# traveller59/second.pytorch

Hardware: AMD Instinct MI355X
Metric: frames/sec VoxelNet fwd (car.fhd, ~16k active voxels) (higher is better)
Workload: dtype bf16; 1 GPU; car.fhd.config VoxelNet forward (voxelise+VFE+SpMiddleFHD+RPNV2+rotated NMS), inference, batch=8 synthetic KITTI clouds/GPU (17000 pts, 16000 voxels each), random-init weights, inputs resident in HBM; parallelism=frame-dp1, launch_mode=graph, graph_branches=1, steps_in_flight=4, rpn_segments_serialized=True, rulebook_numbering=sorted, points_per_frame=17000

## Files before the change

second.pytorch_amd/csrc/indice_conv.hip:

```cpp
#include "common.hpp"
#include <stdlib.h>
#include <type_traits>

namespace sec {

template <typename T> struct Cvt;
template <> struct Cvt<float> {
    static __device__ __forceinline__ float to(float v) { return v; }
    static __device__ __forceinline__ float from(float v) { return v; }
};
template <> struct Cvt<__half> {
    static __device__ __forceinline__ float to(__half v) { return __half2float(v); }
    static __device__ __forceinline__ __half from(float v) { return __float2half_rn(v); }
};
template <> struct Cvt<__hip_bfloat16> {
    static __device__ __forceinline__ float to(__hip_bfloat16 v) { return __bfloat162float(v); }
    static __device__ __forceinline__ __hip_bfloat16 from(float v) { return __float2bfloat16(v); }
};

__device__ __forceinline__ float epilogue(float v, const float *scale, const float *shift, int c, int relu) {
    if (scale) v = __fmul_rn(v, scale[c]);
    if (shift) v = __fadd_rn(v, shift[c]);
    if (relu) v = v > 0.0f ? v : 0.0f;
    return v;
// ... 346 lines not shown
            }
            if (valid) store4<OT>(out + (size_t)row * COUT + c0, v[0], v[1], v[2], v[3]);
        }
    }
}

template <typename T, typename OT, int COUT>
__global__ __launch_bounds__(kBlock) void k_conv_c4(const T *__restrict__ feat, const T *__restrict__ w,
                                                   const int *__restrict__ nbr, int n_out,
                                                   const int *__restrict__ num_out_dev, int kvol,
                                                   const float *__restrict__ scale, const float *__restrict__ shift,
                                                   int relu, OT *__restrict__ out) {
    extern __shared__ __attribute__((aligned(16))) float wl[];
    if (num_out_dev) n_out = *num_out_dev;
    for (int e = threadIdx.x; e < kvol * 4 * COUT; e += kBlock) wl[e] = Cvt<T>::to(w[e]);
    __syncthreads();
    long long o = (long long)blockIdx.x * kBlock + threadIdx.x;
    if (o >= n_out) return;
    float acc[COUT];
#pragma unroll
    for (int c = 0; c < COUT; ++c) acc[c] = 0.0f;
    const int *row = nbr + (size_t)o * kvol;
    for (int k = 0; k < kvol; ++k) {
        int idx = row[k];
        if (idx < 0) continue;
        float f[4];
        if (sizeof(T) == 2) {
            uint2 v = *reinterpret_cast<const uint2 *>(feat + (size_t)idx * 4);
            const T *pv = reinterpret_cast<const T *>(&v);
#pragma unroll
            for (int c = 0; c < 4; ++c) f[c] = Cvt<T>::to(pv[c]);
        } else {
            float4 v = *reinterpret_cast<const float4 *>(feat + (size_t)idx * 4);
            f[0] = v.x; f[1] = v.y; f[2] = v.z; f[3] = v.w;
        }
        const float *wk = wl + k * 4 * COUT;
#pragma unroll
        for (int ci = 0; ci < 4; ++ci)
#pragma unroll
            for (int c = 0; c < COUT; ++c) acc[c] = fmaf(f[ci], wk[ci * COUT + c], acc[c]);
    }
    OT *dst = out + (size_t)o * COUT;
#pragma unroll
    for (int c = 0; c < COUT; ++c) dst[c] = Cvt<OT>::from(epilogue(acc[c], scale, shift, c, relu));
}

#ifdef SEC_CONV_EXPERIMENTS
#include "../../tools/kernel_experiments/indice_conv_experiments.inc"
#endif



typedef __attribute__((address_space(3))) void *lds_ptr_c;
typedef const __attribute__((address_space(1))) void *glb_ptr_c;
template <int N> __device__ __forceinline__ void cwait_vmcnt() { asm volatile("s_waitcnt vmcnt(%0)" ::"n"(N) : "memory"); }
__device__ __forceinline__ void clds_barrier() { asm volatile("s_waitcnt lgkmcnt(0)\n\ts_barrier" ::: "memory"); }

template <typename T, int CIN, int COUT>
struct RowsCfg {
    static constexpr int KS = CIN / 16, NT = (COUT + 31) / 32;
    static constexpr int LPR = CIN / 8;
    static constexpr int RPI = 64 / LPR;
    static constexpr int ND = 32 / RPI;
    static constexpr int BPIECES = KS * NT;
    static constexpr int NBW = BPIECES >= 4 ? BPIECES / 4 : 1;
    static constexpr int L = ND + NBW + 1;
    static constexpr int ASLOT = 32 * LPR, BSLOT = BPIECES * 64;
    static constexpr int RING = 3;
};

typedef float f32x2p __attribute__((ext_vector_type(2)));
template <typename T> __device__ __forceinline__ unsigned pack2_16(float a, float b);
template <> __device__ __forceinline__ unsigned pack2_16<__hip_bfloat16>(float a, float b) {
    typedef __bf16 bf16x2p __attribute__((ext_vector_type(2)));
    const f32x2p v = {a, b};
    return __builtin_bit_cast(unsigned, __builtin_convertvector(v, bf16x2p));
}
template <> __device__ __forceinline__ unsigned pack2_16<__half>(float a, float b) {
    typedef _Float16 f16x2p __attribute__((ext_vector_type(2)));
    const f32x2p v = {a, b};
    return __builtin_bit_cast(unsigned, __builtin_convertvector(v, f16x2p));
}

template <typename T, int COUT, bool FUSED>
__device__ __forceinline__ void rows_store_impl(f32x16 (&acc)[(COUT + 31) / 32], T *__restrict__ out, long long row, bool valid, int h,
                                                const float *__restrict__ aff, bool has_scale, bool has_shift, int relu) {
    if (FUSED) { has_scale = has_shift = true; relu = 1; }
    constexpr int NT = (COUT + 31) / 32, NG = COUT >= 32 ? 4 : COUT / 8;
    static_assert(COUT % 16 == 0, "whole 16-byte runs per half-wave pair");
    T *orow = out + (size_t)row * COUT;
    float4 sc4[NT][NG], sh4[NT][NG];
#pragma unroll
    for (int t = 0; t < NT; ++t)
#pragma unroll
        for (int g = 0; g < NG; ++g) {
            const int c = t * 32 + 8 * g + 4 * h;
            if (has_scale) sc4[t][g] = *reinterpret_cast<const float4 *>(aff + c);
            if (has_shift) sh4[t][g] = *reinterpret_cast<const float4 *>(aff + COUT + c);
        }
#pragma unroll
    for (int t = 0; t < NT; ++t) {
        unsigned lo[NG], hi[NG];
#pragma unroll
        for (int g = 0; g < NG; ++g) {
            const float sc[4] = {sc4[t][g].x, sc4[t][g].y, sc4[t][g].z, sc4[t][g].w};
            const float sh[4] = {sh4[t][g].x, sh4[t][g].y, sh4[t][g].z, sh4[t][g].w};
            float v4[4];
#pragma unroll
            for (int j = 0; j < 4; ++j) v4[j] = epilogue_v(acc[t][4 * g + j], sc[j], sh[j], has_scale, has_shift, relu);
            lo[g] = pack2_16<T>(v4[0], v4[1]);
            hi[g] = pack2_16<T>(v4[2], v4[3]);
        }
#pragma unroll
        for (int pr = 0; pr < NG / 2; ++pr) {
            const auto sx = __builtin_amdgcn_permlane32_swap(lo[2 * pr], lo[2 * pr + 1], false, false);
            const auto sy = __builtin_amdgcn_permlane32_swap(hi[2 * pr], hi[2 * pr + 1], false, false);
            if (valid) *reinterpret_cast<uint4 *>(orow + t * 32 + 8 * (2 * pr + h)) = make_uint4(sx[0], sy[0], sx[1], sy[1]);
        }
    }
}
template <typename T, int COUT>
__device__ __forceinline__ void rows_store(f32x16 (&acc)[(COUT + 31) / 32], T *__restrict__ out, long long row, bool valid, int h,
                                           const float *__restrict__ aff, bool has_scale, bool has_shift, int relu) {
    if (has_scale && has_shift && relu) rows_store_impl<T, COUT, true>(acc, out, row, valid, h, aff, true, true, 1);
    else rows_store_impl<T, COUT, false>(acc, out, row, valid, h, aff, has_scale, has_shift, relu);
}

template <int COUT>
__device__ __forceinline__ void rows_stage_affine(float *aff, const float *__restrict__ scale, const float *__restrict__ shift) {
    const int c = threadIdx.x;
    if (c < COUT) {
        if (scale) aff[c] = scale[c];
        if (shift) aff[COUT + c] = shift[c];
    }
}

#ifdef SEC_CONV_TIMELINE
#define SEC_RTL(...) __VA_ARGS__
#else
#define SEC_RTL(...)
#endif

#ifdef SEC_CONV_EXPERIMENTS
#include "../../tools/kernel_experiments/indice_conv_rows_ab.inc"
#endif

typedef unsigned int u32x4_t __attribute__((ext_vector_type(4)));
constexpr int kBalWgs = 256;
#if defined(__HIP_DEVICE_COMPILE__) && defined(SEC_PACKED_F32_EXEMPTION)
#define SEC_PACKED_F32_OK __attribute__((target("packed-fp32-ops")))
#else
#define SEC_PACKED_F32_OK
#endif
template <typename T, int CIN, int COUT, int KVOL, int DIST, int WAVES, int MINW, int FL>
SEC_PACKED_F32_OK __global__ __launch_bounds__(WAVES * 64, MINW) void k_conv_rows_buf(const T *__restrict__ feat, long long feat_bytes,
                                                                   const T *__restrict__ packed, const int *__restrict__ nbr,
                                                                   int n_out, const int *__restrict__ num_out_dev,
                                                                   const float *__restrict__ scale, const float *__restrict__ shift,
                                                                   int relu, T *__restrict__ out) {
    using C = RowsCfg<T, CIN, COUT>;
    constexpr int NBW = (C::BPIECES + WAVES - 1) / WAVES;
    constexpr int ROWB = CIN * (int)sizeof(T);
    constexpr bool STAGE = (FL & 1) != 0, PIPE = (FL & 2) != 0;
    constexpr bool ALLW = (FL & 64) != 0;
    constexpr bool LAZY = (FL & 128) != 0 && STAGE && !ALLW;
    constexpr bool SKEW = (FL & 32) != 0 && WAVES == 8 && PIPE;
    const bool early = SKEW && __builtin_amdgcn_readfirstlane((int)threadIdx.x >> 8) != 0;
    constexpr int TBL16 = 32 * KVOL / 4;
    static_assert(NBW >= 1 && NBW <= 2, "one or two weight pieces per wave");
    static_assert(C::KS <= 4, "up to four 16-channel k-steps per row");
    static_assert(!STAGE || (32 * KVOL) % 4 == 0, "tile table in whole 16-byte pieces");
    static_assert(!ALLW || (STAGE && PIPE), "the all-weights form stages its tables and double-buffers its B fragments");
    constexpr bool WIN3 = (FL & 512) != 0;
    static_assert(!WIN3 || (STAGE && !PIPE && !ALLW && KVOL % 3 == 0 && DIST <= 3), "window form: non-pipelined, 3 offsets per window");
    constexpr int LBUF = ALLW ? (KVOL * C::BSLOT > WAVES * TBL16 ? KVOL * C::BSLOT : WAVES * TBL16) : 1;
    __shared__ __attribute__((aligned(16))) uint4 lbuf[LBUF];
    __shared__ __attribute__((aligned(16))) uint4 bring[ALLW ? 1 : (WIN3 ? 6 : 3)][ALLW ? 1 : C::BSLOT];
    __shared__ __attribute__((aligned(16))) float aff[2 * COUT];
    __shared__ __attribute__((aligned(16))) u32x4_t stage[(STAGE && !ALLW) ? WAVES : 1][(STAGE && !ALLW) ? TBL16 : 1];
    rows_stage_affine<COUT>(aff, scale, shift);
    const int n_cap = n_out;
    if (num_out_dev) n_out = *num_out_dev;
    const int lane = threadIdx.x & 63, w = threadIdx.x >> 6;
    const int r = lane & 31, h = lane >> 5;
    constexpr bool BAL = (FL & 2048) != 0;
    int rw = 32;
    if constexpr (BAL) {
        const int per_wg = (n_out + kBalWgs - 1) / kBalWgs;
        rw = ((per_wg + WAVES - 1) / WAVES + 3) & ~3;
        rw = rw < 4 ? 4 : (rw > 32 ? 32 : rw);
    }
    int bid = blockIdx.x;
    if (relu & 0x10000) {
        const int nact = (int)(((long long)n_out + rw * WAVES - 1) / (rw * WAVES));
        const int per = (nact + 7) >> 3;
        bid = (bid & 7) * per + (bid >> 3);
        if ((int)(blockIdx.x >> 3) >= per) return;
    }
    relu &= 1;
    if ((long long)bid * (rw * WAVES) >= n_out) return;
    const long long row = (long long)bid * (rw * WAVES) + w * rw + r;
    const bool valid = row < n_out && r < rw;
    SEC_RTL(long long *tl = g_timeline; long long tl0 = 0, tl1 = 0, tl2 = 0; if (tl) tl0 = clock64();)
    const __amdgpu_buffer_rsrc_t rsrc = __builtin_amdgcn_make_buffer_rsrc(const_cast<T *>(feat), 0, (int)feat_bytes, 0x00020000);
    const int piece0 = (w * NBW) % C::BPIECES;
    const u32x4_t *wpv = reinterpret_cast<const u32x4_t *>(packed) + (size_t)piece0 * 64 + lane;
    unsigned off[KVOL];
    if constexpr (STAGE) {
        const long long tile_row0 = (long long)bid * (rw * WAVES) + w * rw;
        const long long tbl_bytes = (long long)n_cap * KVOL * 4;
        const int *tile = nbr + tile_row0 * KVOL;
        const long long left = tbl_bytes - tile_row0 * KVOL * 4;
        const __amdgpu_buffer_rsrc_t trs = __builtin_amdgcn_make_buffer_rsrc(
            const_cast<int *>(left > 0 ? tile : nbr), 0, (int)(left <= 0 ? 0 : (left < 32 * KVOL * 4 ? left : 32 * KVOL * 4)), 0x00020000);
        u32x4_t *stg = ALLW ? reinterpret_cast<u32x4_t *>(lbuf) + w * TBL16 : &stage[w][0];
#pragma unroll
        for (int i = 0; i < (TBL16 + 63) / 64; ++i) {
            const int p16 = i * 64 + lane;
            if (p16 < TBL16) stg[p16] = __builtin_amdgcn_raw_buffer_load_b128(trs, p16 * 16, 0, 0);
        }
        __builtin_amdgcn_wave_barrier();
        const int *mine = reinterpret_cast<const int *>(stg) + r * KVOL;
        if constexpr (!LAZY) {
#pragma unroll
            for (int k = 0; k < KVOL; ++k) {
                const int t = valid ? mine[k] : -1;
                off[k] = t >= 0 ? (unsigned)t * ROWB + h * 16 : 0x80000000u;
            }
        }
    } else {
        const int *nrow = nbr + (size_t)(valid ? row : 0) * KVOL;
#pragma unroll
        for (int k = 0; k < KVOL; ++k) {
            const int t = valid ? nrow[k] : -1;
            off[k] = t >= 0 ? (unsigned)t * ROWB + h * 16 : 0x80000000u;
        }
    }
#ifdef SEC_CONV_ABLATIONS
    if constexpr ((FL & 4) != 0) {
#pragma unroll
        for (int k = 0; k < KVOL; ++k) off[k] = 0x80000000u;
    }
    if constexpr ((FL & 8) != 0) {
#pragma unroll
        for (int k = 0; k < KVOL; ++k) off[k] = (unsigned)__shfl((int)off[k], lane & ~3, 64);
    }
    if constexpr ((FL & 16) != 0) {
#pragma unroll
        for (int k = 0; k < KVOL; ++k) off[k] = h * 16;
    }
#endif
    SEC_RTL(if (tl) { cwait_vmcnt<0>(); tl1 = clock64(); })
    f32x16 acc[C::NT];
#pragma unroll
    for (int t = 0; t < C::NT; ++t)
#pragma unroll
        for (int i = 0; i < 16; ++i) acc[t][i] = 0.0f;
    u32x4_t areg[DIST][C::KS];
    if constexpr (ALLW) {
#define SEC_FETCH_A(k)                                                                                                \
    {                                                                                                                 \
        areg[(k) % DIST][0] = __builtin_amdgcn_raw_buffer_load_b128(rsrc, off[k], 0, 0);                              \
        if (C::KS > 1) areg[(k) % DIST][1 % C::KS] = __builtin_amdgcn_raw_buffer_load_b128(rsrc, off[k] + 32, 0, 0);  \
        if (C::KS > 2) areg[(k) % DIST][2 % C::KS] = __builtin_amdgcn_raw_buffer_load_b128(rsrc, off[k] + 64, 0, 0);  \
        if (C::KS > 3) areg[(k) % DIST][3 % C::KS] = __builtin_amdgcn_raw_buffer_load_b128(rsrc, off[k] + 96, 0, 0);  \
    }
#pragma unroll
        for (int k = 0; k < DIST && k < KVOL; ++k) SEC_FETCH_A(k)
        __syncthreads();
        {
            const uint4 *pk = reinterpret_cast<const uint4 *>(packed);
            for (int i = threadIdx.x; i < KVOL * C::BSLOT; i += WAVES * 64) lbuf[i] = pk[i];
        }
        __syncthreads();
        uint4 bf[2][C::KS * C::NT];
#pragma unroll
        for (int i = 0; i < C::KS * C::NT; ++i) bf[0][i] = lbuf[i * 64 + lane];
#pragma unroll
        for (int k = 0; k < KVOL; ++k) {
            if (k + 1 < KVOL) {
#pragma unroll
                for (int i = 0; i < C::KS * C::NT; ++i) bf[(k + 1) & 1][i] = lbuf[(k + 1) * C::BSLOT + i * 64 + lane];
            }
            __builtin_amdgcn_sched_barrier(0);
#pragma unroll
            for (int s = 0; s < C::KS; ++s) {
                const uint4 a = __builtin_bit_cast(uint4, areg[k % DIST][s]);
#pragma unroll
                for (int t = 0; t < C::NT; ++t) acc[t] = Mfma<T>::run(bf[k & 1][s * C::NT + t], a, acc[t]);
            }
            __builtin_amdgcn_sched_barrier(0);
            if (k + DIST < KVOL) SEC_FETCH_A(k + DIST)
        }
#undef SEC_FETCH_A
        SEC_RTL(if (tl) tl2 = clock64();)
        rows_store<T, COUT>(acc, out, row, valid, h, aff, scale != nullptr, shift != nullptr, relu);
        return;
    }
    u32x4_t wr0[DIST], wr1[DIST];
    u32x4_t *bslot = reinterpret_cast<u32x4_t *>(&bring[0][piece0 * 64 + lane]);
    const int *lazy_tbl = reinterpret_cast<const int *>(&stage[(STAGE && !ALLW) ? w : 0][0]) + r * KVOL;
    auto off_of = [&](int k) -> unsigned {
        if constexpr (LAZY) {
            const int t = valid ? lazy_tbl[k] : -1;
#ifdef SEC_CONV_ABLATIONS
            if constexpr ((FL & 4) != 0) return 0x80000000u;
            if constexpr ((FL & 16) != 0) return t >= 0 ? (unsigned)(h * 16) : 0x80000000u;
#endif
            return t >= 0 ? (unsigned)t * ROWB + h * 16 : 0x80000000u;
        } else {
            return off[k];
        }
    };
#define SEC_FETCH(k)                                                                                                  \
    {                                                                                                                 \
        const unsigned o_ = off_of(k);                                                                                \
        wr0[(k) % DIST] = wpv[(size_t)(k) * C::BSLOT];                                                                \
        if (NBW > 1) wr1[(k) % DIST] = wpv[(size_t)(k) * C::BSLOT + 64];                                              \
        areg[(k) % DIST][0] = __builtin_amdgcn_raw_buffer_load_b128(rsrc, o_, 0, 0);                                  \
        if (C::KS > 1) areg[(k) % DIST][1 % C::KS] = __builtin_amdgcn_raw_buffer_load_b128(rsrc, o_ + 32, 0, 0);      \
        if (C::KS > 2) areg[(k) % DIST][2 % C::KS] = __builtin_amdgcn_raw_buffer_load_b128(rsrc, o_ + 64, 0, 0);      \
        if (C::KS > 3) areg[(k) % DIST][3 % C::KS] = __builtin_amdgcn_raw_buffer_load_b128(rsrc, o_ + 96, 0, 0);      \
    }
#define SEC_WPUT(k)                                                                                                   \
    {                                                                                                                 \
        bslot[((k) % 3) * C::BSLOT] = wr0[(k) % DIST];                                                                \
        if (NBW > 1) bslot[((k) % 3) * C::BSLOT + 64] = wr1[(k) % DIST];                                              \
    }
#pragma unroll
    for (int k = 0; k < DIST && k < KVOL; ++k) SEC_FETCH(k)
    SEC_RTL(long long ts_wait = 0, ts_comp = 0, ts_issue = 0;)
    if constexpr (WIN3) {
        u32x4_t ww0[3], ww1[3];
#define SEC_GFETCH(k)                                                                                                 \
    {                                                                                                                 \
        const unsigned o_ = off_of(k);                                                                                \
        areg[(k) % DIST][0] = __builtin_amdgcn_raw_buffer_load_b128(rsrc, o_, 0, 0);                                  \
        if (C::KS > 1) areg[(k) % DIST][1 % C::KS] = __builtin_amdgcn_raw_buffer_load_b128(rsrc, o_ + 32, 0, 0);      \
        if (C::KS > 2) areg[(k) % DIST][2 % C::KS] = __builtin_amdgcn_raw_buffer_load_b128(rsrc, o_ + 64, 0, 0);      \
        if (C::KS > 3) areg[(k) % DIST][3 % C::KS] = __builtin_amdgcn_raw_buffer_load_b128(rsrc, o_ + 96, 0, 0);      \
    }
#ifdef SEC_CONV_ABLATIONS
#define SEC_WLOAD(g)                                                                                                  \
    {                                                                                                                 \
        _Pragma("unroll") for (int j_ = 0; j_ < 3; ++j_) {                                                            \
            if constexpr ((FL & 4096) != 0) { ww0[j_] = u32x4_t{(unsigned)lane, 0u, 0u, 0u}; if (NBW > 1) ww1[j_] = ww0[j_]; }  \
            else {                                                                                                    \
            ww0[j_] = wpv[(size_t)(3 * (g) + j_) * C::BSLOT];                                                         \
            if (NBW > 1) ww1[j_] = wpv[(size_t)(3 * (g) + j_) * C::BSLOT + 64];                                       \
            }                                                                                                         \
        }                                                                                                             \
    }
#else
#define SEC_WLOAD(g)                                                                                                  \
    {                                                                                                                 \
        _Pragma("unroll") for (int j_ = 0; j_ < 3; ++j_) {                                                            \
            ww0[j_] = wpv[(size_t)(3 * (g) + j_) * C::BSLOT];                                                         \
            if (NBW > 1) ww1[j_] = wpv[(size_t)(3 * (g) + j_) * C::BSLOT + 64];                                       \
        }                                                                                                             \
    }
#endif
#define SEC_WSTORE(g)                                                                                                 \
    {                                                                                                                 \
        _Pragma("unroll") for (int j_ = 0; j_ < 3; ++j_) {                                                            \
            bslot[((((g) & 1) * 3) + j_) * C::BSLOT] = ww0[j_];                                                       \
            if (NBW > 1) bslot[((((g) & 1) * 3) + j_) * C::BSLOT + 64] = ww1[j_];                                     \
        }                                                                                                             \
    }
        SEC_WLOAD(0)
#pragma unroll
        for (int k = 0; k < DIST && k < KVOL; ++k) SEC_GFETCH(k)
        SEC_WSTORE(0)
        if (KVOL > 3) SEC_WLOAD(1)
#pragma unroll
        for (int g = 0; g < KVOL / 3; ++g) {
            __syncthreads();
#pragma unroll
            for (int j = 0; j < 3; ++j) {
                const int k = 3 * g + j;
                uint4 bf[C::KS * C::NT];
#pragma unroll
                for (int i = 0; i < C::KS * C::NT; ++i) bf[i] = bring[(g & 1) * 3 + j][i * 64 + lane];
                __builtin_amdgcn_sched_barrier(0);
#pragma unroll
                for (int s2 = 0; s2 < C::KS; ++s2) {
                    const uint4 a = __builtin_bit_cast(uint4, areg[k % DIST][s2]);
#pragma unroll
                    for (int t = 0; t < C::NT; ++t) acc[t] = Mfma<T>::run(bf[s2 * C::NT + t], a, acc[t]);
                }
                __builtin_amdgcn_sched_barrier(0);
                if (k + DIST < KVOL) SEC_GFETCH(k + DIST)
            }
            if (g + 1 < KVOL / 3) {
                SEC_WSTORE(g + 1)
                if (g + 2 < KVOL / 3) SEC_WLOAD(g + 2)
            }
        }
#undef SEC_GFETCH
#undef SEC_WLOAD
#undef SEC_WSTORE
    } else if constexpr (!PIPE) {
        SEC_WPUT(0)
#pragma unroll
        for (int k = 0; k < KVOL; ++k) {
            SEC_RTL(long long s0 = 0, s1 = 0, s2 = 0; if (tl) s0 = clock64();)
            if (k + 1 < KVOL) SEC_WPUT(k + 1)
            __syncthreads();
            SEC_RTL(if (tl) s1 = clock64();)
            uint4 bf[C::KS * C::NT];
#pragma unroll
            for (int i = 0; i < C::KS * C::NT; ++i) bf[i] = bring[k % 3][i * 64 + lane];
            __builtin_amdgcn_sched_barrier(0);
#pragma unroll
            for (int s = 0; s < C::KS; ++s) {
                const uint4 a = __builtin_bit_cast(uint4, areg[k % DIST][s]);
#pragma unroll
                for (int t = 0; t < C::NT; ++t) acc[t] = Mfma<T>::run(bf[s * C::NT + t], a, acc[t]);
            }
            __builtin_amdgcn_sched_barrier(0);
            SEC_RTL(if (tl) s2 = clock64();)
            if (k + DIST < KVOL) SEC_FETCH(k + DIST)
            SEC_RTL(if (tl) { const long long s3 = clock64(); ts_wait += s1 - s0; ts_comp += s2 - s1; ts_issue += s3 - s2; })
        }
    } else {
        static_assert(!PIPE || DIST >= 3, "W[k+2] must have left the ring before its registers are refilled");
        uint4 bf[2][C::KS * C::NT];
        SEC_WPUT(0)
        if (KVOL > 1) SEC_WPUT(1)
        __syncthreads();
#pragma unroll
        for (int i = 0; i < C::KS * C::NT; ++i) bf[0][i] = bring[0][i * 64 + lane];
#pragma unroll
        for (int k = 0; k < KVOL; ++k) {
            if (k + 2 < KVOL) SEC_WPUT(k + 2)
            if (k + 1 < KVOL) {
                __syncthreads();
#pragma unroll
                for (int i = 0; i < C::KS * C::NT; ++i) bf[(k + 1) & 1][i] = bring[(k + 1) % 3][i * 64 + lane];
            }
            __builtin_amdgcn_sched_barrier(0);
            if constexpr (SKEW) {
                if (early && k >= 1 && k - 1 + DIST < KVOL) SEC_FETCH(k - 1 + DIST)
                __builtin_amdgcn_sched_barrier(0);
            }
#pragma unroll
            for (int s = 0; s < C::KS; ++s) {
                const uint4 a = __builtin_bit_cast(uint4, areg[k % DIST][s]);
#pragma unroll
                for (int t = 0; t < C::NT; ++t) acc[t] = Mfma<T>::run(bf[k & 1][s * C::NT + t], a, acc[t]);
            }
            __builtin_amdgcn_sched_barrier(0);
            if (!(SKEW && early) && k + DIST < KVOL) SEC_FETCH(k + DIST)
        }
    }
#undef SEC_FETCH
#undef SEC_WPUT
    SEC_RTL(if (tl) tl2 = clock64();)
    rows_store<T, COUT>(acc, out, row, valid, h, aff, scale != nullptr, shift != nullptr, relu);
#ifdef SEC_CONV_TIMELINE
    if (tl && lane == 0) {
        long long *rec = tl + ((size_t)blockIdx.x * WAVES + w) * 8;
        rec[0] = tl0; rec[1] = tl1; rec[2] = tl2; rec[3] = clock64(); rec[4] = ts_wait; rec[5] = ts_issue; rec[6] = ts_comp;
        rec[7] = __builtin_amdgcn_s_getreg((4 << 11) | 20);
    }
#endif
}

template <typename T, int CIN, int COUT, int DIST, int WAVES, int MINW, int FL, int KVOL = 27>
static void launch_rows_buf(const void *feat, long long n_feat, const void *packed, const int *nbr, int n_out, const int *num_out_dev,
                            const float *scale, const float *shift, int relu, void *out, hipStream_t st) {
    set_last_kernel("k_conv_rows_buf<%s, %d, %d, %d, %d, %d, %d, %d>", dtype_name<T>(), CIN, COUT, KVOL, DIST, WAVES, MINW, FL);
    int blocks = div_up(n_out, 32 * WAVES);
    if ((FL & 2048) != 0 && blocks < kBalWgs) blocks = kBalWgs;
    const int xcd = rows_xcd_order();
    if (xcd) blocks = (blocks + 7) / 8 * 8 + 8;
    hipLaunchKernelGGL((k_conv_rows_buf<T, CIN, COUT, KVOL, DIST, WAVES, MINW, FL>), dim3(blocks), dim3(WAVES * 64), 0, st,
                       (const T *)feat, n_feat * CIN * (long long)sizeof(T), (const T *)packed, nbr, n_out, num_out_dev, scale, shift,
                       (relu & 1) | (xcd << 16), (T *)out);
}

#ifdef SEC_CONV_EXPERIMENTS
#include "../../tools/kernel_experiments/indice_conv_rows_r06.inc"
#endif

#ifdef SEC_CONV_EXPERIMENTS
#include "../../tools/kernel_experiments/indice_conv_rows_r03.inc"
#endif

template <typename T>
__global__ __launch_bounds__(kBlock) void k_pack_weight_c4(const T *__restrict__ w, int cout, T *__restrict__ packed) {
    const int g = blockIdx.x * kBlock + threadIdx.x;
    if (g >= 7 * 64 * 8) return;
    const int e = g & 7, lane = (g >> 3) & 63, s_ = g >> 9;
    const int K = s_ * 16 + (lane >> 5) * 8 + e, kk = K >> 2, ci = K & 3, c = lane & 31;
    packed[g] = (kk < 27 && c < cout) ? w[((size_t)kk * 4 + ci) * cout + c] : Cvt<T>::from(0.0f);
}

template <typename T, int COUT>
__global__ __launch_bounds__(kBlock) void k_conv_c4_mfma(const T *__restrict__ feat, long long feat_bytes, const T *__restrict__ packed,
                                                        const int *__restrict__ nbr, int n_out, const int *__restrict__ num_out_dev,
                                                        const float *__restrict__ scale, const float *__restrict__ shift, int relu,
                                                        T *__restrict__ out) {
    constexpr int KVOL = 27, TBL16 = 32 * KVOL / 4;
    __shared__ __attribute__((aligned(16))) u32x4_t stage[4][TBL16];
    __shared__ __attribute__((aligned(16))) float aff[2 * COUT];
    rows_stage_affine<COUT>(aff, scale, shift);
    const int n_cap = n_out;
    if (num_out_dev) n_out = *num_out_dev;
    const int lane = threadIdx.x & 63, w = threadIdx.x >> 6;
    const int r = lane & 31, h = lane >> 5;
    int bid = blockIdx.x;
    if (relu & 0x10000) {
        const int per = (int)((((long long)n_out + 127) / 128 + 7) >> 3);
        bid = (int)(blockIdx.x >> 3) < per ? (bid & 7) * per + (bid >> 3) : 0x3fffff;
    }
    relu &= 1;
    const long long tile_row0 = (long long)bid * 128 + w * 32;
    const long long row = tile_row0 + r;
    const bool valid = row < n_out;
    if (tile_row0 < n_out) {
        const __amdgpu_buffer_rsrc_t rsrc = __builtin_amdgcn_make_buffer_rsrc(const_cast<T *>(feat), 0, (int)feat_bytes, 0x00020000);
        const long long left = ((long long)n_cap - tile_row0) * KVOL * 4;
        const __amdgpu_buffer_rsrc_t trs = __builtin_amdgcn_make_buffer_rsrc(
            const_cast<int *>(nbr + tile_row0 * KVOL), 0, (int)(left < 32 * KVOL * 4 ? left : 32 * KVOL * 4), 0x00020000);
#pragma unroll
        for (int i = 0; i < (TBL16 + 63) / 64; ++i) {
            const int p16 = i * 64 + lane;
            if (p16 < TBL16) stage[w][p16] = __builtin_amdgcn_raw_buffer_load_b128(trs, p16 * 16, 0, 0);
        }
        __builtin_amdgcn_wave_barrier();
        const int *mine = reinterpret_cast<const int *>(&stage[w][0]) + r * KVOL;
        const u32x4_t *wp = reinterpret_cast<const u32x4_t *>(packed) + lane;
        typedef unsigned int u32x2_t __attribute__((ext_vector_type(2)));
        u32x4_t bfr[7];
        u32x2_t lo[7], hi[7];
#pragma unroll
        for (int s = 0; s < 7; ++s) {
            bfr[s] = wp[s * 64];
            const int k0 = 4 * s + 2 * h, k1 = k0 + 1;
            const int t0 = valid ? mine[k0] : -1;
            const int t1 = (valid && k1 < KVOL) ? mine[k1 < KVOL ? k1 : 0] : -1;
            lo[s] = __builtin_amdgcn_raw_buffer_load_b64(rsrc, t0 >= 0 ? (unsigned)t0 * 8u : 0x80000000u, 0, 0);
            hi[s] = __builtin_amdgcn_raw_buffer_load_b64(rsrc, t1 >= 0 ? (unsigned)t1 * 8u : 0x80000000u, 0, 0);
        }
        f32x16 acc[1];
#pragma unroll
        for (int i = 0; i < 16; ++i) acc[0][i] = 0.0f;
#pragma unroll
        for (int s = 0; s < 7; ++s) {
            const uint4 a = make_uint4(lo[s].x, lo[s].y, hi[s].x, hi[s].y);
            acc[0] = Mfma<T>::run(__builtin_bit_cast(uint4, bfr[s]), a, acc[0]);
        }
        __syncthreads();
        rows_store<T, COUT>(acc, out, row, valid, h, aff, scale != nullptr, shift != nullptr, relu);
    } else {
        __syncthreads();
    }
}

static int g_variant_override = -1;
static int g_fp32_mode = 0;
static int conv_variant() {
    if (g_variant_override >= 0) return g_variant_override;
    return 1;
}

enum { PLAN_GENERIC = 0, PLAN_TILED = 1, PLAN_C4 = 2, PLAN_MFMA_WAVE = 3, PLAN_MFMA_SK = 4, PLAN_MFMA_SKS = 5, PLAN_ROWS = 6,
       PLAN_ROWS_COMPACT = 7, PLAN_ROWS_TOUCH = 8, PLAN_ROWS_COMPACT_TOUCH = 9, PLAN_ROWS_REG = 10, PLAN_ROWS_BUF = 11, PLAN_C4_MFMA = 12, PLAN_ROWS_M2 = 13, PLAN_ROWS_LDS = 14, PLAN_ROWS_KS = 15, PLAN_EXPERIMENT = 99 };

static int rows_min() {
    return 40000;
}
constexpr int kRowsMinSmall = 8192;
static int rows_footprint() {
    return 0;
}
static int m2_auto() { return 0; }
static bool ks_auto() {
    static int v = -1;
    if (v < 0) { const char *e = getenv("SEC_CONV_KS"); v = e ? atoi(e) != 0 : 0; }
    return v != 0;
}
static bool rows_balance() { return true; }
static bool buf_shape(int cin, int cout, int kvol) {
    if (kvol == 3) return cin == 64 && cout == 64;
    if (kvol != 27) return false;
    return (cin == 16 && (cout == 16 || cout == 32)) || (cin == 32 && (cout == 32 || cout == 64)) || (cin == 64 && cout == 64);
}

static int rows_plan(int cin, int cout, int kvol, int n_out, bool same_dtype) {
    if (!same_dtype) return 0;
    const int v = conv_variant();
    if (buf_shape(cin, cout, kvol)) {
#ifdef SEC_CONV_EXPERIMENTS
        if (cin == 64 && cout == 64 && kvol == 27 && v == 46) return PLAN_ROWS_LDS;
        if (cin == 64 && cout == 64 && kvol == 27 && (v == 41 || v == 42 || v == 43 || (v == 1 && m2_auto() && n_out >= rows_min())))
            return PLAN_ROWS_M2;
#endif
#ifdef SEC_CONV_EXPERIMENTS
        if (cin == 64 && cout == 64 && kvol == 27 && (v == 50 || (v >= 71 && v <= 73) || (v == 1 && n_out >= kRowsMinSmall && n_out < rows_min() && ks_auto()))) return PLAN_ROWS_KS;
#endif
        if (v == 22 || (((v >= 16 && v <= 28) || v == 44 || v == 45 || (v >= 60 && v <= 67)) && cin == 64 && cout == 64 && kvol == 27)) return PLAN_ROWS_BUF;
        if (v >= 36 && v <= 40) return PLAN_ROWS_BUF;
        if (v == 1 && n_out >= rows_min()) return PLAN_ROWS_BUF;
        if (v == 1 && cin == 64 && cout == 64 && kvol == 27 && n_out >= kRowsMinSmall) return PLAN_ROWS_BUF;
    }
#ifdef SEC_CONV_EXPERIMENTS
    if (kvol != 27 || !(cin == 64 || cin == 32) || !(cout == 64 || cout == 32)) return 0;
    if (cin == 64) {
        if (v == 10) return PLAN_ROWS_COMPACT;
        if (v == 11) return PLAN_ROWS_TOUCH;
        if (v == 12) return PLAN_ROWS_COMPACT_TOUCH;
        if (v >= 13 && v <= 15 && cout == 64) return PLAN_ROWS_REG;
    }
    if (v == 9) return PLAN_ROWS;
#endif
    return 0;
}

#ifdef SEC_CONV_EXPERIMENTS
template <typename T>
static void launch_rows_lds(const void *feat, long long n_feat, const void *packed, const int *nbr, int n_out, const int *num_out_dev,
                            const float *scale, const float *shift, int relu, void *out, hipStream_t st) {
    set_last_kernel("k_conv_rows_lds<%s>", dtype_name<T>());
    hipLaunchKernelGGL((k_conv_rows_lds<T>), dim3(div_up(n_out, 256)), dim3(256), 0, st, (const T *)feat,
                       n_feat * 64 * (long long)sizeof(T), (const T *)packed, nbr, n_out, num_out_dev, scale, shift, relu, (T *)out);
}

#endif
template <typename T, typename OT, int CIN, int COUT>
static void launch_mfma(const void *feat, long long n_feat, const void *packed, const int *nbr, int n_out, const int *num_out_dev,
                        int kvol, const float *scale, const float *shift, int relu, void *out, hipStream_t st) {
    constexpr int MT = 1;
    if constexpr (std::is_same<T, OT>::value && CIN <= 64 && COUT <= 64 && (COUT >= CIN) ) {
        const int rp = feat ? rows_plan(CIN, COUT, kvol, n_out, true) : 0;
#ifdef SEC_CONV_EXPERIMENTS
        if constexpr (CIN == 64 && COUT == 64) {
            if (rp == PLAN_ROWS_M2 && n_feat * CIN * (long long)sizeof(T) < 0x7fffffffll) {
                launch_rows_m2<T>(feat, n_feat, packed, nbr, n_out, num_out_dev, scale, shift, relu, out, st);
                return;
            }
            if (rp == PLAN_ROWS_LDS && n_feat * CIN * (long long)sizeof(T) < 0x7fffffffll) {
                launch_rows_lds<T>(feat, n_feat, packed, nbr, n_out, num_out_dev, scale, shift, relu, out, st);
                return;
            }
        }
#endif
#ifdef SEC_CONV_EXPERIMENTS
        if constexpr (CIN == 64 && COUT == 64) {
            if (rp == PLAN_ROWS_KS && n_feat * CIN * (long long)sizeof(T) < 0x7fffffffll) {
#ifdef SEC_CONV_ABLATIONS
                if (conv_variant() == 71) { launch_rows_ks<T, 4, 3, 2>(feat, n_feat, packed, nbr, n_out, num_out_dev, scale, shift, relu, out, st); return; }
                if (conv_variant() == 72) { launch_rows_ks<T, 4, 3, 1>(feat, n_feat, packed, nbr, n_out, num_out_dev, scale, shift, relu, out, st); return; }
                if (conv_variant() == 73) { launch_rows_ks<T, 4, 3, 3>(feat, n_feat, packed, nbr, n_out, num_out_dev, scale, shift, relu, out, st); return; }
#endif
                launch_rows_ks<T, 4, 3>(feat, n_feat, packed, nbr, n_out, num_out_dev, scale, shift, relu, out, st);
                return;
            }
        }
#endif
        if (rp == PLAN_ROWS_BUF && n_feat * CIN * (long long)sizeof(T) < 0x7fffffffll) {
#define SEC_BUF(D, W, FLG, KV) launch_rows_buf<T, CIN, COUT, D, W, 2, FLG, KV>(feat, n_feat, packed, nbr, n_out, num_out_dev, scale, shift, relu, out, st)
            if (kvol == 3) {
                if constexpr (CIN == 64 && COUT == 64) { SEC_BUF(3, 8, 3, 3); return; }
            } else {
#ifdef SEC_CONV_EXPERIMENTS
                if constexpr (CIN <= 32) {
                    switch (conv_variant()) {
                    case 36: SEC_BUF(6, 8, 3, 27); return;
                    case 37: SEC_BUF(8, 8, 3, 27); return;
                    case 38: SEC_BUF(12, 8, 3, 27); return;
                    case 39: if constexpr (COUT <= 32) { SEC_BUF(4, 8, 3 + 64, 27); return; } break;
                    case 40: if constexpr (COUT <= 32) { SEC_BUF(6, 8, 3 + 64, 27); return; } break;
                    default: break;
                    }
                }
                if constexpr (CIN == 64 && COUT == 64) {
                    switch (conv_variant()) {
                    case 16: SEC_BUF(4, 4, 0, 27); return;
                    case 17: SEC_BUF(4, 4, 1, 27); return;
                    case 18: SEC_BUF(4, 4, 2, 27); return;
                    case 19: SEC_BUF(4, 4, 3, 27); return;
                    case 20: SEC_BUF(5, 4, 3, 27); return;
                    case 21: SEC_BUF(5, 8, 3, 27); return;
                    case 23: SEC_BUF(6, 4, 3, 27); return;
                    case 27: SEC_BUF(5, 8, 3 + 32, 27); return;
                    case 28: SEC_BUF(6, 8, 3 + 32, 27); return;
#ifdef SEC_CONV_ABLATIONS
                    case 24: SEC_BUF(4, 8, 3 + 4, 27); return;
                    case 25: SEC_BUF(4, 8, 3 + 8, 27); return;
                    case 26: SEC_BUF(4, 8, 3 + 16, 27); return;
                    case 60: launch_rows_buf<T, CIN, COUT, 3, 4, 2, 1 + 128 + 512 + 2048 + 4096, 27>(feat, n_feat, packed, nbr, n_out, num_out_dev, scale, shift, relu, out, st); return;
                    case 61: launch_rows_buf<T, CIN, COUT, 3, 4, 2, 1 + 128 + 512 + 2048 + 4, 27>(feat, n_feat, packed, nbr, n_out, num_out_dev, scale, shift, relu, out, st); return;
                    case 62: launch_rows_buf<T, CIN, COUT, 3, 4, 2, 1 + 128 + 512 + 2048 + 4096 + 4, 27>(feat, n_feat, packed, nbr, n_out, num_out_dev, scale, shift, relu, out, st); return;
                    case 63: launch_rows_buf<T, CIN, COUT, 3, 8, 3, 1 + 128 + 512 + 2048 + 4096, 27>(feat, n_feat, packed, nbr, n_out, num_out_dev, scale, shift, relu, out, st); return;
                    case 64: launch_rows_buf<T, CIN, COUT, 3, 8, 3, 1 + 128 + 512 + 2048 + 4, 27>(feat, n_feat, packed, nbr, n_out, num_out_dev, scale, shift, relu, out, st); return;
                    case 65: launch_rows_buf<T, CIN, COUT, 3, 8, 3, 1 + 128 + 512 + 2048 + 4096 + 4, 27>(feat, n_feat, packed, nbr, n_out, num_out_dev, scale, shift, relu, out, st); return;
                    case 66: launch_rows_buf<T, CIN, COUT, 3, 4, 2, 1 + 128 + 512 + 2048, 27>(feat, n_feat, packed, nbr, n_out, num_out_dev, scale, shift, relu, out, st); return;
                    case 67: launch_rows_buf<T, CIN, COUT, 3, 8, 3, 1 + 128 + 512 + 2048, 27>(feat, n_feat, packed, nbr, n_out, num_out_dev, scale, shift, relu, out, st); return;
                    case 44: launch_rows_buf<T, CIN, COUT, 3, 8, 3, 1 + 128 + 512 + 4, 27>(feat, n_feat, packed, nbr, n_out, num_out_dev, scale, shift, relu, out, st); return;
                    case 45: launch_rows_buf<T, CIN, COUT, 3, 8, 3, 1 + 128 + 512 + 16, 27>(feat, n_feat, packed, nbr, n_out, num_out_dev, scale, shift, relu, out, st); return;
#endif
                    default: break;
                    }
                }
#endif
                const bool bal = rows_balance();
                if constexpr (CIN <= 32 && COUT <= 32) { if (bal) { SEC_BUF(6, 8, 3 + 64 + 2048, 27); } else { SEC_BUF(6, 8, 3 + 64, 27); } }
                else if constexpr (CIN == 64 && COUT == 64) {
#define SEC_BUFM(D, W, M, FLG) launch_rows_buf<T, CIN, COUT, D, W, M, FLG, 27>(feat, n_feat, packed, nbr, n_out, num_out_dev, scale, shift, relu, out, st)
                    if (n_out < rows_min() && conv_variant() == 1) {
                        if (rows_footprint() == 4) { SEC_BUF(4, 4, 3, 27); }
                        else if (bal) { SEC_BUFM(3, 4, 2, 1 + 128 + 512 + 2048); }
                        else { SEC_BUFM(3, 4, 2, 1 + 128 + 512); }
                    } else if (rows_footprint() == 1) { SEC_BUF(4, 8, 3, 27); }
                    else if (rows_footprint() == 3) { SEC_BUFM(3, 8, 3, 1 + 128); }
                    else if (bal) { SEC_BUFM(3, 8, 3, 1 + 128 + 512 + 2048); }
                    else { SEC_BUFM(3, 8, 3, 1 + 128 + 512); }
#undef SEC_BUFM
                } else if (bal) { SEC_BUF(4, 8, 3 + 2048, 27); }
                else { SEC_BUF(4, 8, 3, 27); }
                return;
            }
#undef SEC_BUF
        }
    }
#ifdef SEC_CONV_EXPERIMENTS
    if constexpr (std::is_same<T, OT>::value && (CIN == 64 || CIN == 32) && (COUT == 64 || COUT == 32)) {
        const int rp = feat ? rows_plan(CIN, COUT, kvol, n_out, true) : 0;
        if constexpr (CIN == 64) {
            if (rp == PLAN_ROWS_COMPACT) { launch_rows<T, CIN, COUT, 32>(feat, packed, nbr, n_out, num_out_dev, kvol, scale, shift, relu, out, st); return; }
            if (rp == PLAN_ROWS_TOUCH) { launch_rows<T, CIN, COUT, 64>(feat, packed, nbr, n_out, num_out_dev, kvol, scale, shift, relu, out, st); return; }
            if (rp == PLAN_ROWS_COMPACT_TOUCH) { launch_rows<T, CIN, COUT, 96>(feat, packed, nbr, n_out, num_out_dev, kvol, scale, shift, relu, out, st); return; }
            if constexpr (COUT == 64) {
                if (rp == PLAN_ROWS_REG) {
                    const int v = conv_variant();
                    if (v == 13) launch_rows_reg<T, CIN, COUT, 4, 2>(feat, packed, nbr, n_out, num_out_dev, scale, shift, relu, out, st);
                    else if (v == 14) launch_rows_reg<T, CIN, COUT, 2, 3>(feat, packed, nbr, n_out, num_out_dev, scale, shift, relu, out, st);
                    else launch_rows_reg<T, CIN, COUT, 5, 2>(feat, packed, nbr, n_out, num_out_dev, scale, shift, relu, out, st);
                    return;
                }
            }
        }
        if (rp == PLAN_ROWS) {
            launch_rows<T, CIN, COUT, 0>(feat, packed, nbr, n_out, num_out_dev, kvol, scale, shift, relu, out, st);
            return;
        }
#ifdef SEC_CONV_ABLATIONS
        if (conv_variant() >= 91 && conv_variant() <= 96 && kvol == 27 && feat && CIN == 64 && COUT == 64) {
            switch (conv_variant()) {
            case 91: launch_rows<T, CIN, COUT, 1>(feat, packed, nbr, n_out, num_out_dev, kvol, scale, shift, relu, out, st); break;
            case 92: launch_rows<T, CIN, COUT, 2>(feat, packed, nbr, n_out, num_out_dev, kvol, scale, shift, relu, out, st); break;
            case 93: launch_rows<T, CIN, COUT, 4>(feat, packed, nbr, n_out, num_out_dev, kvol, scale, shift, relu, out, st); break;
            case 94: launch_rows<T, CIN, COUT, 8>(feat, packed, nbr, n_out, num_out_dev, kvol, scale, shift, relu, out, st); break;
            case 95: launch_rows<T, CIN, COUT, 16>(feat, packed, nbr, n_out, num_out_dev, kvol, scale, shift, relu, out, st); break;
            default: launch_rows<T, CIN, COUT, 3>(feat, packed, nbr, n_out, num_out_dev, kvol, scale, shift, relu, out, st); break;
            }
            return;
        }
#endif
    }
#endif
#ifdef SEC_CONV_EXPERIMENTS
    if (conv_variant() == 2 && kvol == 27) {
        hipLaunchKernelGGL((k_conv_mfma_lds<T, OT, CIN, COUT, 27>), dim3(div_up(n_out, 128)), dim3(kBlock), 0, st,
                           (const T *)feat, (const T *)packed, nbr, n_out, num_out_dev, scale, shift, relu, (OT *)out);
        return;
    }
    if (conv_variant() == 7 && kvol == 27 && CIN <= 64 && CIN >= 32) {
        launch_wlds_fl<T, OT, CIN, COUT>(feat, packed, nbr, n_out, num_out_dev, scale, shift, relu, out, st);
        return;
    }
    if ((conv_variant() == 6 || conv_variant() == 7) && kvol == 27 && CIN <= 64) {
        launch_wlds<T, OT, CIN, COUT>(feat, packed, nbr, n_out, num_out_dev, scale, shift, relu, out, st);
        return;
    }
#endif
    if (conv_variant() == 8 || ((conv_variant() == 1 || conv_variant() == 29) && COUT <= 32)) {
        hipLaunchKernelGGL((k_conv_mfma_sks<T, OT, CIN, COUT, 4>), dim3((div_up(n_out, 32) + 7) / 8 * 8, (COUT + 31) / 32),
                           dim3(256), 0, st, (const T *)feat, (const T *)packed, nbr, n_out, num_out_dev, kvol, scale, shift,
                           relu, (OT *)out);
        return;
    }
#ifdef SEC_CONV_EXPERIMENTS
    if (conv_variant() == 3 && kvol == 27) {
        hipLaunchKernelGGL((k_conv_mfma_lds2<T, OT, CIN, COUT, 27>), dim3(div_up(n_out, 128)), dim3(kBlock), 0, st,
                           (const T *)feat, (const T *)packed, nbr, n_out, num_out_dev, scale, shift, relu, (OT *)out);
        return;
    }
    if (conv_variant() == 4 || conv_variant() == 5) {
        if (conv_variant() == 4)
            hipLaunchKernelGGL((k_conv_mfma_skm<T, OT, CIN, COUT, 2>), dim3(div_up(n_out, 64)), dim3(kBlock), 0, st,
                               (const T *)feat, (const T *)packed, nbr, n_out, num_out_dev, kvol, scale, shift, relu, (OT *)out);
        else
            hipLaunchKernelGGL((k_conv_mfma_skm<T, OT, CIN, COUT, 1>), dim3(div_up(n_out, 32)), dim3(kBlock), 0, st,
                               (const T *)feat, (const T *)packed, nbr, n_out, num_out_dev, kvol, scale, shift, relu, (OT *)out);
        return;
    }
#endif
    if (conv_variant() >= 1) {
        constexpr int NW = 4;
        hipLaunchKernelGGL((k_conv_mfma_sk<T, OT, CIN, COUT, NW>), dim3((div_up(n_out, 32) + 7) / 8 * 8), dim3(NW * 64), 0, st,
                           (const T *)feat, (const T *)packed, nbr, n_out, num_out_dev, kvol, scale, shift,
                           relu | (conv_swizzle() << 16), (OT *)out);
        return;
    }
    int rows_per_block = (kBlock / 64) * 32 * MT;
    hipLaunchKernelGGL((k_conv_mfma<T, OT, CIN, COUT, MT>), dim3(div_up(n_out, rows_per_block)), dim3(kBlock), 0, st,
                       (const T *)feat, (const T *)packed, nbr, n_out, num_out_dev, kvol, scale, shift, relu, (OT *)out);
}

template <typename T, typename OT>
static bool dispatch_mfma(int cin, int cout, const void *feat, long long n_feat, const void *packed, const int *nbr, int n_out,
                          const int *num_out_dev, int kvol, const float *scale, const float *shift, int relu, void *out,
                          hipStream_t st) {
#define SEC_CASE(CI, CO)                                                                                         \
    if (cin == CI && cout == CO) {                                                                               \
        launch_mfma<T, OT, CI, CO>(feat, n_feat, packed, nbr, n_out, num_out_dev, kvol, scale, shift, relu, out, st); \
        return true;                                                                                             \
    }
    SEC_CASE(16, 16) SEC_CASE(16, 32) SEC_CASE(32, 32) SEC_CASE(32, 64) SEC_CASE(64, 64) SEC_CASE(64, 128)
    SEC_CASE(128, 128) SEC_CASE(16, 64) SEC_CASE(64, 32) SEC_CASE(32, 16) SEC_CASE(128, 64)
#undef SEC_CASE
    return false;
}

template <int CIN, int COUT, int WAVES>
__global__ __launch_bounds__(WAVES * 64) void k_conv_rows_x3_f32(const float *__restrict__ feat, const float *__restrict__ w,
                                                                const int *__restrict__ nbr, int n_out, const int *__restrict__ num_out_dev,
                                                                int kvol, int w_t, int mirror, const float *__restrict__ scale,
                                                                const float *__restrict__ shift, int relu, float *__restrict__ out) {
    static_assert(CIN % 16 == 0 && COUT % 32 == 0, "16-channel k-steps, 32-column MFMA tiles");
    constexpr int KS = CIN / 16, NT = COUT / 32, ROWS = WAVES * 32, NTH = WAVES * 64;
    constexpr int PIECES = KS * NT * 64;
    constexpr int PPT = (PIECES + NTH - 1) / NTH;
    __shared__ __attribute__((aligned(16))) uint4 sB[2][2][PIECES];
    __shared__ int s_nbr[ROWS * 27];
    if (num_out_dev) n_out = *num_out_dev;
    const int tid = threadIdx.x, wave = tid >> 6, lane = tid & 63, r = lane & 31, h = lane >> 5;
    const long long base = (long long)blockIdx.x * ROWS;
    if (base >= n_out) return;
    {
        const long long lim = ((long long)n_out - base) * kvol;
        const int *src = nbr + base * kvol;
        for (int e = tid; e < ROWS * kvol; e += NTH) s_nbr[e] = e < lim ? src[e] : -1;
    }
    float wreg[PPT][8];
    auto load_w = [&](int k) {
        const float *wk = w + (size_t)(mirror ? kvol - 1 - k : k) * CIN * COUT;
#pragma unroll
        for (int q = 0; q < PPT; ++q) {
            const int p = q * NTH + tid;
            if (PIECES % NTH != 0 && p >= PIECES) break;
            const int l = p & 63, st = p >> 6, t = st % NT, sidx = st / NT;
            const int ci = sidx * 16 + (l >> 5) * 8, co = t * 32 + (l & 31);
            if (w_t) {
                const float4 a = *reinterpret_cast<const float4 *>(wk + (size_t)co * CIN + ci);
                const float4 b = *reinterpret_cast<const float4 *>(wk + (size_t)co * CIN + ci + 4);
                wreg[q][0] = a.x; wreg[q][1] = a.y; wreg[q][2] = a.z; wreg[q][3] = a.w;
                wreg[q][4] = b.x; wreg[q][5] = b.y; wreg[q][6] = b.z; wreg[q][7] = b.w;
            } else {
#pragma unroll
                for (int e = 0; e < 8; ++e) wreg[q][e] = wk[(size_t)(ci + e) * COUT + co];
            }
        }
    };
    auto split8 = [](const float (&v)[8], uint4 &hi, uint4 &lo) {
        const unsigned h0 = pack2_16<__hip_bfloat16>(v[0], v[1]), h1 = pack2_16<__hip_bfloat16>(v[2], v[3]);
        const unsigned h2 = pack2_16<__hip_bfloat16>(v[4], v[5]), h3 = pack2_16<__hip_bfloat16>(v[6], v[7]);
// ... 1122 lines not shown
```

Baseline: 21300 frames/s.

## Share neighbor feature rows across adjacent lanes via DPP in 3x3x3 rows conv

Adds an XSH mode to the buffered rows submanifold conv. When an adjacent output row (lane r±1) gathers the same input row for a side kernel offset as this row's centre offset, the load is skipped and the A fragment is taken from the neighbouring lane with DPP wave shifts. The refill schedule is reordered so the centre offset of each window of three is fetched first. The goal is to cut redundant global/buffer gather traffic, in exchange for extra DPP moves, selects and a sharing bitmask per lane. It is enabled by default for the 32-channel and the 64-channel 8-wave paths, with an env var or variant override to switch it.

```diff
diff --git a/second.pytorch_amd/csrc/indice_conv.hip b/second.pytorch_amd/csrc/indice_conv.hip
--- a/second.pytorch_amd/csrc/indice_conv.hip
+++ b/second.pytorch_amd/csrc/indice_conv.hip
@@ -522,6 +522,14 @@
 #else
 #define SEC_PACKED_F32_OK
 #endif
+template <int CTRL> __device__ __forceinline__ int rows_lane_shift(int v) {
+    return __builtin_amdgcn_mov_dpp(v, CTRL, 0xf, 0xf, true);
+}
+constexpr int kDppWaveShl1 = 0x130, kDppWaveShr1 = 0x138;
+template <bool LEFT> __device__ __forceinline__ bool rows_xshare(int t, int c, int r) {
+    const int n = rows_lane_shift<LEFT ? kDppWaveShr1 : kDppWaveShl1>(c);
+    return t >= 0 && t == n && (LEFT ? r > 0 : r < 31);
+}
 template <typename T, int CIN, int COUT, int KVOL, int DIST, int WAVES, int MINW, int FL>
 SEC_PACKED_F32_OK __global__ __launch_bounds__(WAVES * 64, MINW) void k_conv_rows_buf(const T *__restrict__ feat, long long feat_bytes,
                                                                    const T *__restrict__ packed, const int *__restrict__ nbr,
@@ -542,6 +550,7 @@
     static_assert(!STAGE || (32 * KVOL) % 4 == 0, "tile table in whole 16-byte pieces");
     static_assert(!ALLW || (STAGE && PIPE), "the all-weights form stages its tables and double-buffers its B fragments");
     constexpr bool WIN3 = (FL & 512) != 0;
+    constexpr bool XSH = (FL & 8192) != 0 && STAGE && KVOL == 27 && DIST >= 3 && (ALLW || (WIN3 && LAZY));
     static_assert(!WIN3 || (STAGE && !PIPE && !ALLW && KVOL % 3 == 0 && DIST <= 3), "window form: non-pipelined, 3 offsets per window");
     constexpr int LBUF = ALLW ? (KVOL * C::BSLOT > WAVES * TBL16 ? KVOL * C::BSLOT : WAVES * TBL16) : 1;
     __shared__ __attribute__((aligned(16))) uint4 lbuf[LBUF];
@@ -576,6 +585,7 @@
     const int piece0 = (w * NBW) % C::BPIECES;
     const u32x4_t *wpv = reinterpret_cast<const u32x4_t *>(packed) + (size_t)piece0 * 64 + lane;
     unsigned off[KVOL];
+    unsigned shm = 0;
     if constexpr (STAGE) {
         const long long tile_row0 = (long long)bid * (rw * WAVES) + w * rw;
         const long long tbl_bytes = (long long)n_cap * KVOL * 4;
@@ -594,7 +604,13 @@
         if constexpr (!LAZY) {
 #pragma unroll
             for (int k = 0; k < KVOL; ++k) {
-                const int t = valid ? mine[k] : -1;
+                int t = valid ? mine[k] : -1;
+                if constexpr (XSH) {
+                    if (k % 3 != 1) {
+                        const int c = valid ? mine[k - k % 3 + 1] : -1;
+                        if (k % 3 == 0 ? rows_xshare<true>(t, c, r) : rows_xshare<false>(t, c, r)) { shm |= 1u << (2 * (k / 3) + (k % 3) / 2); t = -1; }
+                    }
+                }
                 off[k] = t >= 0 ? (unsigned)t * ROWB + h * 16 : 0x80000000u;
             }
         }
@@ -627,6 +643,31 @@
 #pragma unroll
         for (int i = 0; i < 16; ++i) acc[t][i] = 0.0f;
     u32x4_t areg[DIST][C::KS];
+    auto afrag = [&](int k, int s) __attribute__((always_inline)) -> uint4 {
+        u32x4_t a = areg[k % DIST][s];
+        if constexpr (XSH) {
+            if (k % 3 != 1) {
+                const bool sh = ((shm >> (2 * (k / 3) + (k % 3) / 2)) & 1u) != 0;
+                const u32x4_t c = areg[(k - k % 3 + 1) % DIST][s];
+#pragma unroll
+                for (int i = 0; i < 4; ++i) {
+                    const int n = k % 3 == 0 ? rows_lane_shift<kDppWaveShr1>((int)c[i]) : rows_lane_shift<kDppWaveShl1>((int)c[i]);
+                    a[i] = sh ? (unsigned)n : a[i];
+                }
+            }
+        }
+        return __builtin_bit_cast(uint4, a);
+    };
+#define SEC_XSH_REFILL(k, FETCH)                                                                                      \
+    if constexpr (XSH) {                                                                                              \
+        if ((k) % 3 == 0) { if ((k) + DIST < KVOL) FETCH((k) + DIST) }                                                \
+        else if ((k) % 3 == 2) {                                                                                      \
+            if ((k) - 1 + DIST < KVOL) FETCH((k) - 1 + DIST)                                                          \
+            if ((k) + DIST < KVOL) FETCH((k) + DIST)                                                                  \
+        }                                                                                                             \
+    } else {                                                                                                          \
+        if ((k) + DIST < KVOL) FETCH((k) + DIST)                                                                      \
+    }
     if constexpr (ALLW) {
 #define SEC_FETCH_A(k)                                                                                                \
     {                                                                                                                 \
@@ -655,12 +696,12 @@
             __builtin_amdgcn_sched_barrier(0);
 #pragma unroll
             for (int s = 0; s < C::KS; ++s) {
-                const uint4 a = __builtin_bit_cast(uint4, areg[k % DIST][s]);
+                const uint4 a = afrag(k, s);
 #pragma unroll
                 for (int t = 0; t < C::NT; ++t) acc[t] = Mfma<T>::run(bf[k & 1][s * C::NT + t], a, acc[t]);
             }
             __builtin_amdgcn_sched_barrier(0);
-            if (k + DIST < KVOL) SEC_FETCH_A(k + DIST)
+            SEC_XSH_REFILL(k, SEC_FETCH_A)
         }
 #undef SEC_FETCH_A
         SEC_RTL(if (tl) tl2 = clock64();)
@@ -672,7 +713,13 @@
     const int *lazy_tbl = reinterpret_cast<const int *>(&stage[(STAGE && !ALLW) ? w : 0][0]) + r * KVOL;
     auto off_of = [&](int k) -> unsigned {
         if constexpr (LAZY) {
-            const int t = valid ? lazy_tbl[k] : -1;
+            int t = valid ? lazy_tbl[k] : -1;
+            if constexpr (XSH) {
+                if (k % 3 != 1) {
+                    const int c = valid ? lazy_tbl[k - k % 3 + 1] : -1;
+                    if (k % 3 == 0 ? rows_xshare<true>(t, c, r) : rows_xshare<false>(t, c, r)) { shm |= 1u << (2 * (k / 3) + (k % 3) / 2); t = -1; }
+                }
+            }
 #ifdef SEC_CONV_ABLATIONS
             if constexpr ((FL & 4) != 0) return 0x80000000u;
             if constexpr ((FL & 16) != 0) return t >= 0 ? (unsigned)(h * 16) : 0x80000000u;
@@ -697,8 +744,10 @@
         bslot[((k) % 3) * C::BSLOT] = wr0[(k) % DIST];                                                                \
         if (NBW > 1) bslot[((k) % 3) * C::BSLOT + 64] = wr1[(k) % DIST];                                              \
     }
-#pragma unroll
-    for (int k = 0; k < DIST && k < KVOL; ++k) SEC_FETCH(k)
+    if constexpr (!(WIN3 && XSH)) {
+#pragma unroll
+        for (int k = 0; k < DIST && k < KVOL; ++k) SEC_FETCH(k)
+    }
     SEC_RTL(long long ts_wait = 0, ts_comp = 0, ts_issue = 0;)
     if constexpr (WIN3) {
         u32x4_t ww0[3], ww1[3];
@@ -754,12 +803,12 @@
                 __builtin_amdgcn_sched_barrier(0);
 #pragma unroll
                 for (int s2 = 0; s2 < C::KS; ++s2) {
-                    const uint4 a = __builtin_bit_cast(uint4, areg[k % DIST][s2]);
+                    const uint4 a = afrag(k, s2);
 #pragma unroll
                     for (int t = 0; t < C::NT; ++t) acc[t] = Mfma<T>::run(bf[s2 * C::NT + t], a, acc[t]);
                 }
                 __builtin_amdgcn_sched_barrier(0);
-                if (k + DIST < KVOL) SEC_GFETCH(k + DIST)
+                SEC_XSH_REFILL(k, SEC_GFETCH)
             }
             if (g + 1 < KVOL / 3) {
                 SEC_WSTORE(g + 1)
@@ -825,6 +874,7 @@
     }
 #undef SEC_FETCH
 #undef SEC_WPUT
+#undef SEC_XSH_REFILL
     SEC_RTL(if (tl) tl2 = clock64();)
     rows_store<T, COUT>(acc, out, row, valid, h, aff, scale != nullptr, shift != nullptr, relu);
 #ifdef SEC_CONV_TIMELINE
@@ -931,6 +981,7 @@
 static int g_variant_override = -1;
 static int g_fp32_mode = 0;
 static int conv_variant() {
+    if (g_variant_override >= 80 && g_variant_override <= 83) return g_variant_override <= 81 ? 1 : 22;
     if (g_variant_override >= 0) return g_variant_override;
     return 1;
 }
@@ -951,6 +1002,14 @@
     if (v < 0) { const char *e = getenv("SEC_CONV_KS"); v = e ? atoi(e) != 0 : 0; }
     return v != 0;
 }
+static int xshare_mode() {
+    if (g_variant_override == 80 || g_variant_override == 82) return 0;
+    if (g_variant_override == 81 || g_variant_override == 83) return 1;
+    static int v = -2;
+    if (v == -2) { const char *e = getenv("SEC_CONV_XSHARE"); v = e ? (atoi(e) != 0) : -1; }
+    return v;
+}
+constexpr bool kXshare32 = true, kXshare64w8 = true, kXshare64w4 = false;
 static bool rows_balance() { return true; }
 static bool buf_shape(int cin, int cout, int kvol) {
     if (kvol == 3) return cin == 64 && cout == 64;
@@ -1076,15 +1135,23 @@
                 }
 #endif
                 const bool bal = rows_balance();
-                if constexpr (CIN <= 32 && COUT <= 32) { if (bal) { SEC_BUF(6, 8, 3 + 64 + 2048, 27); } else { SEC_BUF(6, 8, 3 + 64, 27); } }
+                const int xsm = xshare_mode();
+                if constexpr (CIN <= 32 && COUT <= 32) {
+                    if constexpr (CIN == 32) {
+                        if (bal && (xsm < 0 ? kXshare32 : xsm != 0)) { SEC_BUF(6, 8, 3 + 64 + 2048 + 8192, 27); return; }
+                    }
+                    if (bal) { SEC_BUF(6, 8, 3 + 64 + 2048, 27); } else { SEC_BUF(6, 8, 3 + 64, 27); }
+                }
                 else if constexpr (CIN == 64 && COUT == 64) {
 #define SEC_BUFM(D, W, M, FLG) launch_rows_buf<T, CIN, COUT, D, W, M, FLG, 27>(feat, n_feat, packed, nbr, n_out, num_out_dev, scale, shift, relu, out, st)
                     if (n_out < rows_min() && conv_variant() == 1) {
                         if (rows_footprint() == 4) { SEC_BUF(4, 4, 3, 27); }
+                        else if (bal && (xsm < 0 ? kXshare64w4 : xsm != 0)) { SEC_BUFM(3, 4, 2, 1 + 128 + 512 + 2048 + 8192); }
                         else if (bal) { SEC_BUFM(3, 4, 2, 1 + 128 + 512 + 2048); }
                         else { SEC_BUFM(3, 4, 2, 1 + 128 + 512); }
                     } else if (rows_footprint() == 1) { SEC_BUF(4, 8, 3, 27); }
                     else if (rows_footprint() == 3) { SEC_BUFM(3, 8, 3, 1 + 128); }
+                    else if (bal && (xsm < 0 ? kXshare64w8 : xsm != 0)) { SEC_BUFM(3, 8, 3, 1 + 128 + 512 + 2048 + 8192); }
                     else if (bal) { SEC_BUFM(3, 8, 3, 1 + 128 + 512 + 2048); }
                     else { SEC_BUFM(3, 8, 3, 1 + 128 + 512); }
 #undef SEC_BUFM
```

Result: faster. 21640 frames/s (median of 6 runs) (+1.6%).
